# Unsigned-Long/slam-tricks

Hardware: AMD Instinct MI355X
Metric: LM iterations/sec + residuals/sec, 1k-cam/100k-pt BA (higher is better)
Workload: dtype f64

## Files before the change

slam-tricks_amd/csrc/dense_chol.hip:

```cpp
#include <algorithm>
#include <atomic>
#include <cstdlib>
#include <map>
#include <mutex>
#include <queue>
#include <string>
#include <vector>

#include "common.hpp"

namespace stba {

constexpr int NB = CHOL_NB;
#ifndef MEGA_WAIT_SLEEP
#define MEGA_WAIT_SLEEP 1
#endif
#ifndef MEGA_POLL_SLEEP
#define MEGA_POLL_SLEEP 16
#endif

typedef double double4v __attribute__((ext_vector_type(4)));

__global__ void chol_pad_kernel(double* __restrict__ A, int lda, int n, const double* __restrict__ rhs) {
    const int r = n + blockIdx.x;
// ... 455 lines not shown
        for (int p = 0; p < 2; ++p)
#pragma unroll
            for (int h = 0; h < 2; ++h) {
                const int row = lrow + 16 * (w + 4 * p);
                const int k = 2 * (lkp + 4 * h);
                if (p < PA) ga[p < PA ? p : 0][h] = *reinterpret_cast<const double2*>(&A[(size_t)(row_i + row) * lda + k0 + kc * 16 + k]);
                gb[p][h] = *reinterpret_cast<const double2*>(&A[(size_t)(row_j + row) * lda + k0 + kc * 16 + k]);
            }
    };
    auto lstore = [&](int buf) {
#pragma unroll
        for (int p = 0; p < 2; ++p)
#pragma unroll
            for (int h = 0; h < 2; ++h) {
                const int rb = w + 4 * p;
                const int k = 2 * (lkp + 4 * h);
                if (p < PA) {
                    const int posa = (((k >> 2) * RBA + rb) << 6) + ((k & 3) << 4) + lrow;
                    sA[buf][posa] = ga[p < PA ? p : 0][h].x;
                    sA[buf][posa + 16] = ga[p < PA ? p : 0][h].y;
                }
                const int posb = (((k >> 2) * 8 + rb) << 6) + ((k & 3) << 4) + lrow;
                sB[buf][posb] = gb[p][h].x;
                sB[buf][posb + 16] = gb[p][h].y;
            }
    };
    gload(0);
    lstore(0);
    __syncthreads();
    constexpr int KC = NB / 16;
    for (int kc = 0; kc < KC; ++kc) {
        const int buf = kc & 1;
        if (kc + 1 < KC) gload(kc + 1);
#pragma unroll
        for (int kq = 0; kq < 4; ++kq) {
            double a[MB], b[NBK];
#pragma unroll
            for (int m = 0; m < MB; ++m) a[m] = -sA[buf][((kq * RBA + wr * MB + m) << 6) + lane];
#pragma unroll
            for (int n = 0; n < NBK; ++n) b[n] = sB[buf][((kq * 8 + wc * NBK + n) << 6) + lane];
#pragma unroll
            for (int m = 0; m < MB; ++m)
#pragma unroll
                for (int n = 0; n < NBK; ++n)
                    acc[m][n] = __builtin_amdgcn_mfma_f64_16x16x4f64(a[m], b[n], acc[m][n], 0, 0, 0);
        }
        if (kc + 1 < KC) lstore(buf ^ 1);
        __syncthreads();
    }
#pragma unroll
    for (int m = 0; m < MB; ++m)
#pragma unroll
        for (int n = 0; n < NBK; ++n)
#pragma unroll
            for (int r = 0; r < 4; ++r) {
                const int row = row_i + wr * (MB * 16) + m * 16 + (lane >> 4) + 4 * r;
                const int col = row_j + wc * (NBK * 16) + n * 16 + (lane & 15);
                A[(size_t)row * lda + col] = acc[m][n][r];
            }
}

static void launch_syrk(double* A, int lda, int k0, int tile_mode, int tiles128, hipStream_t st) {
    const bool use64 = tiles128 < 1000000;
    if (use64) hipLaunchKernelGGL(chol_syrk_kernel<64>, dim3(2 * tiles128), dim3(256), 0, st, A, lda, k0, tile_mode);
    else hipLaunchKernelGGL(chol_syrk_kernel<128>, dim3(tiles128), dim3(256), 0, st, A, lda, k0, tile_mode);
}

enum { TASK_D = 0, TASK_T = 1, TASK_TI = 2, TASK_U = 3, TASK_UQ = 4, TASK_TU = 5 };

constexpr int MEGA_MAX_Q = 16;
struct MegaArgs {
    double* A; int lda; int n; int nblk;
    const int4* tasks;
    int nq;
    int lstart[MEGA_MAX_Q + 1];
    signed char xcc_queue[16];
    int* sync;
    double* linv; size_t linv_stride;
    double* vbuf; int nwide;
    long long spin_limit;
    int* flag;
    long long* trace;
};
constexpr int MEGA_SYNC_HDR = MEGA_MAX_Q + 1;
constexpr int MEGA_ABORT = MEGA_MAX_Q;
constexpr int MEGA_SMEM_BYTES = 128 * 1024;
constexpr int MEGA_PREDRAW_NB = 2;

__device__ __forceinline__ int xcc_id() {
    unsigned v;
    asm volatile("s_getreg_b32 %0, hwreg(HW_REG_XCC_ID)" : "=s"(v));
    return (int)(v & 15u);
}
__global__ void xcc_probe_kernel(int* out) {
    if (threadIdx.x == 0) out[blockIdx.x] = xcc_id();
}

template <int TM, int KCH = 16>
__device__ __forceinline__ void syrk_tile512(double* __restrict__ A, int lda, int k0, int row_i, int row_j,
                                             double* smem, int t, int kchunks = NB / 16) {
    constexpr int WR = (TM == 128) ? 2 : 1, WC = 8 / WR;
    constexpr int MB = TM / (16 * WR);
    constexpr int NBK = 8 / WC;
    constexpr int RBA = TM / 16;
    constexpr int SA = TM * KCH, SB = 128 * KCH, NH = KCH / 8;
    double* sA = smem;
    double* sB = smem + 2 * SA;
    const int lane = t & 63, w = t >> 6;
    const int wr = w / WC, wc = w % WC;
    double4v acc[MB][NBK];
#pragma unroll
    for (int m = 0; m < MB; ++m)
#pragma unroll
        for (int n = 0; n < NBK; ++n)
#pragma unroll
            for (int r = 0; r < 4; ++r) {
                const int row = row_i + wr * (MB * 16) + m * 16 + (lane >> 4) + 4 * r;
                const int col = row_j + wc * (NBK * 16) + n * 16 + (lane & 15);
                acc[m][n][r] = A[(size_t)row * lda + col];
            }
    double2 ga[NH], gb[NH];
    const int lrow = lane & 15, lkp = lane >> 4;
    const bool stage_a = (RBA == 8) ? true : (w < RBA);
    auto gload = [&](int kc) {
#pragma unroll
        for (int h = 0; h < NH; ++h) {
            const int row = lrow + 16 * w;
            const int k = 2 * (lkp + 4 * h);
            if (stage_a) ga[h] = *reinterpret_cast<const double2*>(&A[(size_t)(row_i + row) * lda + k0 + kc * KCH + k]);
            gb[h] = *reinterpret_cast<const double2*>(&A[(size_t)(row_j + row) * lda + k0 + kc * KCH + k]);
        }
    };
    auto lstore = [&](int buf) {
#pragma unroll
        for (int h = 0; h < NH; ++h) {
            const int k = 2 * (lkp + 4 * h);
            if (stage_a) {
                const int posa = (((k >> 2) * RBA + w) << 6) + ((k & 3) << 4) + lrow;
                sA[buf * SA + posa] = -ga[h].x;
                sA[buf * SA + posa + 16] = -ga[h].y;
            }
            const int posb = (((k >> 2) * 8 + w) << 6) + ((k & 3) << 4) + lrow;
            sB[buf * SB + posb] = gb[h].x;
            sB[buf * SB + posb + 16] = gb[h].y;
        }
    };
    gload(0);
    lstore(0);
    __syncthreads();
    const int KC = kchunks * 16 / KCH;
    auto chunk = [&](int kc, int buf) {
        if (kc + 1 < KC) gload(kc + 1);
#pragma unroll
        for (int kq = 0; kq < KCH / 4; ++kq) {
            double a[MB], b[NBK];
#pragma unroll
            for (int m = 0; m < MB; ++m) a[m] = sA[buf * SA + (((kq * RBA + wr * MB + m) << 6) + lane)];
#pragma unroll
            for (int n = 0; n < NBK; ++n) b[n] = sB[buf * SB + (((kq * 8 + wc * NBK + n) << 6) + lane)];
#pragma unroll
            for (int m = 0; m < MB; ++m)
#pragma unroll
                for (int n = 0; n < NBK; ++n)
                    acc[m][n] = __builtin_amdgcn_mfma_f64_16x16x4f64(a[m], b[n], acc[m][n], 0, 0, 0);
        }
        if (kc + 1 < KC) lstore(buf ^ 1);
// ... 364 lines not shown
    v.nblk = a.nblk;
    v.nrow = a.nblk + 4 * a.nwide;
    v.abortf = a.sync + MEGA_ABORT;
    v.dflag = a.sync + MEGA_SYNC_HDR;
    v.tuflag = v.dflag + a.nblk;
    v.tudone = v.tuflag + a.nblk;
    v.tflag = v.tudone + a.nblk;
    v.ver = v.tflag + a.nblk * v.nrow;
    return v;
}
__device__ __forceinline__ int mega_ldf(const int* p) { return __hip_atomic_load(p, __ATOMIC_RELAXED, __HIP_MEMORY_SCOPE_AGENT); }
__device__ __forceinline__ bool mega_ready(const MegaView& v, const int4 d, bool& tu_dset) {
    const int type = d.x & 0xff, b = d.y, ti = d.z, tj = d.w;
    const int nblk = v.nblk, nrow = v.nrow;
    auto first_panel = [&](int i) { return i < nblk ? 0 : i - nblk; };
    if (type == TASK_D) return mega_ldf(&v.ver[b * nblk + b]) >= 4 * b;
    if (type == TASK_T) {
        const int ve = mega_ldf(&v.ver[ti * nblk + b]), df = mega_ldf(&v.dflag[b]);
        return (ve >= 4 * (b - first_panel(ti))) & (df >= 1);
    }
    if (type == TASK_TI) return mega_ldf(&v.dflag[b]) >= 1;
    if (type == TASK_TU) {
        const int v0 = mega_ldf(&v.ver[(b + 1) * nblk + b]), v1 = mega_ldf(&v.ver[(b + 1) * nblk + b + 1]), df = mega_ldf(&v.dflag[b]);
        tu_dset = df >= 1;
        return (v0 >= 4 * b) & (v1 >= 4 * b);
    }
    const int i = (type == TASK_UQ) ? (ti >> 2) : ti;
    const int nbp = max(1, (d.x >> 16) & 0xff);
    const int f0 = mega_ldf(&v.tflag[b * nrow + i]), f1 = mega_ldf(&v.tflag[b * nrow + tj]), ve = mega_ldf(&v.ver[i * nblk + tj]);
    return (f0 >= 4) & (f1 >= 4) & (ve >= 4 * (b - nbp + 1 - first_panel(i)));
}

struct MegaTicket {
    int mine = -1;
    int4 md;
    bool done = false;
    int m_raw = 0;
    bool m_pending = false;
};
__device__ __forceinline__ int mega_next_task(const MegaArgs& a, const MegaView& v, MegaTicket& tk, int* ticket, int lbeg, int lend, int lane,
                                              bool& ok, bool& tu_dset, long long& t_poll) {
    t_poll = a.trace ? wall_clock64() : 0;
    ok = true;
    if (tk.mine < 0 && !tk.done) {
        if (!tk.m_pending && lane == 0) tk.m_raw = lbeg + atomicAdd(ticket, 1);
        tk.m_pending = false;
        tk.mine = __builtin_amdgcn_readfirstlane(tk.m_raw);
        if (tk.mine >= lend) { tk.mine = -1; tk.done = true; }
        else tk.md = a.tasks[tk.mine];
    }
    int pick = -2;
    if (tk.mine >= 0) {
        const long long t0 = wall_clock64();
        for (;;) {
            if (mega_ready(v, tk.md, tu_dset)) { pick = tk.mine; tk.mine = -1; break; }
            if (mega_ldf(v.abortf) != 0) { ok = false; pick = -1; break; }
            if (wall_clock64() - t0 > a.spin_limit) {
                __hip_atomic_store(v.abortf, 1, __ATOMIC_RELAXED, __HIP_MEMORY_SCOPE_AGENT);
                ok = false; pick = -1;
                break;
            }
            __builtin_amdgcn_s_sleep(MEGA_POLL_SLEEP);
        }
    }
    asm volatile("buffer_inv sc1\n\ts_waitcnt vmcnt(0)" ::: "memory");
    return pick;
}

__global__ __launch_bounds__(512) void chol_mega_kernel(MegaArgs a) {
    extern __shared__ __attribute__((aligned(16))) double smem[];
    __shared__ int s_task, s_ok, s_dset;
    const int t = threadIdx.x;
    const int nblk = a.nblk;
    const MegaView v = mega_view(a);
    int* abortf = v.abortf;
    int* dflag = v.dflag;
    int* tuflag = v.tuflag;
    const int nrow = v.nrow;
    int* tflag = v.tflag;
    int* ver = v.ver;
    auto tile_ptr = [&](int i, int j, int& ld) -> double* {
        if (i < nblk) { ld = a.lda; return a.A + (size_t)i * NB * a.lda + (size_t)j * NB; }
        const int p = i - nblk, qw = p >> 2;
        ld = 4 * NB;
        return a.vbuf + (size_t)qw * (4 * NB) * (4 * NB) + (size_t)(p & 3) * NB * (4 * NB) + (size_t)(j - 4 * qw) * NB;
    };
    auto first_panel = [&](int i) { return i < nblk ? 0 : i - nblk; };
    const int q = a.xcc_queue[xcc_id()];
    if (q < 0) return;
    int* ticket = a.sync + q;
    const int lbeg = a.lstart[q], lend = a.lstart[q + 1];
    MegaTicket tk;
    for (;;) {
        if (t < 64) {
            bool ok, tu_dset = false;
            long long t_poll;
            const int pick = mega_next_task(a, v, tk, ticket, lbeg, lend, t, ok, tu_dset, t_poll);
            if (t == 0) {
                if (a.trace && pick >= 0) {
                    a.trace[8 * (size_t)pick] = blockIdx.x; a.trace[8 * (size_t)pick + 1] = t_poll;
                    a.trace[8 * (size_t)pick + 2] = wall_clock64();
                }
                s_dset = tu_dset ? 1 : 0;
                s_task = pick;
                s_ok = ok ? 1 : 0;
            }
            if (!tk.done && pick >= 0 && (tk.md.x & 0xff) != TASK_TU && ((tk.md.x >> 16) & 0xff) <= MEGA_PREDRAW_NB) {
                if (t == 0) tk.m_raw = lbeg + atomicAdd(ticket, 1);
                tk.m_pending = true;
            }
        }
        __syncthreads();
        if (!s_ok) {
            if (t == 0) atomicExch(a.flag, CHOL_FLAG_TIMEOUT);
            break;
        }
        const int task = s_task;
        if (task < 0) break;
        const int4 d = a.tasks[task];
        const int type = d.x & 0xff, b = d.y, ti = d.z, tj = d.w;
        const int k0 = b * NB;
        int tt = t;
        asm volatile("" : "+v"(tt));
        double* li = a.linv + (size_t)b * a.linv_stride;
        long long* ph = a.trace ? a.trace + 8 * (size_t)task + 4 : nullptr;
        if (type == TASK_D) {
            diag_block2<true>(a.A, a.lda, k0, a.n, a.flag, li + NB * NB, smem, tt, ph);
        } else if (type == TASK_T) {
            const int lane = tt & 63, w = tt >> 6;
            int ldr;
            const bool active = (tj == 0) || (w < 4);
            const int row_in_tile = (tj == 0 ? 16 * w : 64 * (tj - 1) + 16 * (w & 3)) + (lane & 15);
            double* rowp = tile_ptr(ti, b, ldr) + (size_t)row_in_tile * ldr;
            if (!trsm_task512(rowp, false, 0, NB, a.A + (size_t)k0 * a.lda + k0, a.lda, li + NB * NB, smem, tt, ph, &dflag[b], abortf, &s_ok,
                              a.spin_limit, true, active)) {
                if (t == 0) atomicExch(a.flag, CHOL_FLAG_TIMEOUT);
                break;
            }
        } else if (type == TASK_TI) {
            const int lane = tt & 63, w = tt >> 6;
            const int nv = min(NB, (a.lda - 1) - k0);
            int ldr = NB;
            double* base = li;
            if (b < 4 * a.nwide) base = tile_ptr(nblk + b, b, ldr);
            double* rowp = base + (size_t)(16 * w + (lane & 15)) * ldr;
            if (!trsm_task512(rowp, true, 16 * w, nv, a.A + (size_t)k0 * a.lda + k0, a.lda, li + NB * NB, smem, tt, ph, &dflag[b], abortf, &s_ok,
                              a.spin_limit, true)) {
                if (t == 0) atomicExch(a.flag, CHOL_FLAG_TIMEOUT);
                break;
            }
        } else if (type == TASK_U) {
            if (ti < nblk) {
                const int nbp = max(1, (d.x >> 16) & 0xff);
                syrk_tile512<128>(a.A, a.lda, k0 - (nbp - 1) * NB, ti * NB, tj * NB, smem, tt, nbp * (NB / 16));
            } else {
                int ldc, ldi, ldj;
                double* Cb = tile_ptr(ti, tj, ldc);
                const double* Pi = tile_ptr(ti, b, ldi);
                const double* Pj = tile_ptr(tj, b, ldj);
                syrk_tile512_gen<128>(Cb, ldc, Pi, ldi, Pj, ldj, b == first_panel(ti), smem, tt);
            }
        } else if (type == TASK_TU) {
            const bool tu_ok = (tj == 2)
                ? tu4_task512(a.A, a.lda, k0, b + 1, ti, li + NB * NB, smem, tt, ph, &tuflag[b], &ver[(b + 1) * nblk + b + 1], &dflag[b], abortf, &s_ok,
                              a.spin_limit, s_dset != 0)
                : tu_task512(a.A, a.lda, k0, b + 1, ti, li + NB * NB, smem, tt, ph, &tuflag[b], &v.tudone[b], &ver[(b + 1) * nblk + b + 1], &dflag[b], abortf, &s_ok,
                             a.spin_limit, s_dset != 0);
            if (!tu_ok) {
// ... 109 lines not shown
            }
        for (int i = b + 2; i < NBK; ++i) {
            if (b >= THALF_FROM) {
                idT[(size_t)b * NBK + i] = add(TASK_T, b, i, 1, 10.0 * b + 6 + 1e-3 * i);
                idT2[(size_t)b * NBK + i] = add(TASK_T, b, i, 2, 10.0 * b + 6 + 1e-3 * i + 5e-4);
                nodes[(size_t)idT[(size_t)b * NBK + i]].dur = nodes[(size_t)idT2[(size_t)b * NBK + i]].dur = THALF_DUR * DUR[TASK_T];
            } else idT[(size_t)b * NBK + i] = add(TASK_T, b, i, 0, 10.0 * b + 6 + 1e-3 * i);
            if (i <= b + 1 + QROWS || b >= QFROM) {
                for (int q = 0; q < 4; ++q)
                    idUq[((size_t)b * NBK + i) * 4 + q] = add(TASK_UQ, b, i * 4 + q, b + 1, 10.0 * (b + 1) + 2 + 1e-3 * i);
            } else {
                idUq[((size_t)b * NBK + i) * 4] = add(TASK_U, b, i, b + 1, 10.0 * (b + 1) + 2 + 1e-3 * i);
            }
        }
        for (int j = b + 2; j < NBK; ++j) {
            const int lim = j - 2 - BLAG;
            int BJ = BATCH;
            if (FAR > 0 && BATCH > 1 && j - ((b / (2 * BATCH)) * 2 * BATCH + 2 * BATCH - 1) > FAR) BJ = 2 * BATCH;
            const int b0 = (BJ <= 1 || b > lim) ? b : (b / BJ) * BJ, last = (BJ <= 1 || b > lim) ? b : std::min(b0 + BJ - 1, lim);
            if (b != last) continue;
            const int nb = b - b0 + 1;
            for (int i = j; i < NBK; ++i) {
                if (i == j && j == b + 2 && b >= DQ_FROM) {
                    for (int q = 0; q < 4; ++q) {
                        const int id = add(TASK_UQ, b, i * 4 + q, j, 10.0 * j + 1 + 1e-3 * q);
                        idUd[(size_t)b * 4 + q] = id;
                        if (q == 0) idU[((size_t)b * NBK + i) * NBK + j] = id;
                    }
                    continue;
                }
                const int id = add(TASK_U, b, i, j, 10.0 * j + 3 + 1e-3 * i + 1e-6 * b);
                nodes[(size_t)id].tk.x |= nb << 16;
                nodes[(size_t)id].dur += (nb - 1) * DUR_K;
                for (int bb = b0; bb <= b; ++bb) idU[((size_t)bb * NBK + i) * NBK + j] = id;
            }
        }
    }
    auto dep = [&](int from, int to) {
        if (from < 0 || to < 0) return;
        nodes[(size_t)from].succ.push_back(to);
        nodes[(size_t)to].indeg++;
    };
    for (int b = 0; b < NBK; ++b) {
        const int d = idD[(size_t)b];
        if (b > 0)
            for (int q = 0; q < ntu(b - 1); ++q) dep(idTU[(size_t)(b - 1) * MEGA_NTU + q], d);
        dep(d, idTI[(size_t)b]);
        if (b + 1 < NBK)
            for (int q = 0; q < ntu(b); ++q) {
                const int tu = idTU[(size_t)b * MEGA_NTU + q];
                dep(d, tu);
                if (b > 0) {
                    for (int q2 = 0; q2 < 4; ++q2) dep(idUq[((size_t)(b - 1) * NBK + (b + 1)) * 4 + q2], tu);
                    dep(idU[((size_t)(b - 1) * NBK + (b + 1)) * NBK + (b + 1)], tu);
                    for (int q2 = 1; q2 < 4; ++q2) dep(idUd[(size_t)(b - 1) * 4 + q2], tu);
                }
            }
        for (int i = b + 2; i < NBK; ++i) {
            const int t = idT[(size_t)b * NBK + i], t2 = idT2[(size_t)b * NBK + i];
            dep(d, t); dep(d, t2);
            if (b > 0)
                for (int q2 = 0; q2 < 4; ++q2) { const int uu = idUq[((size_t)(b - 1) * NBK + i) * 4 + q2]; dep(uu, t); dep(uu, t2); }
            for (int q = 0; q < 4; ++q) {
                const int uq = idUq[((size_t)b * NBK + i) * 4 + q];
                if (uq < 0) continue;
                dep(t, uq); dep(t2, uq);
                for (int q2 = 0; q2 < ntu(b); ++q2) dep(idTU[(size_t)b * MEGA_NTU + q2], uq);
                if (b > 0) dep(idU[((size_t)(b - 1) * NBK + i) * NBK + (b + 1)], uq);
            }
        }
        for (int j = b + 2; j < NBK; ++j)
            for (int i = j; i < NBK; ++i) {
                const int u0 = idU[((size_t)b * NBK + i) * NBK + j];
                if (nodes[(size_t)u0].tk.y != b) continue;
                const bool split = (nodes[(size_t)u0].tk.x & 0xff) == TASK_UQ;
                for (int q2 = 0; q2 < (split ? 4 : 1); ++q2) {
                    const int u = split ? idUd[(size_t)b * 4 + q2] : u0;
                    for (auto* v : {&idT, &idT2}) { dep((*v)[(size_t)b * NBK + i], u); if (j != i) dep((*v)[(size_t)b * NBK + j], u); }
                    const int nbp = split ? 1 : std::max(1, (nodes[(size_t)u].tk.x >> 16) & 0xff);
                    if (b - nbp >= 0) dep(idU[((size_t)(b - nbp) * NBK + i) * NBK + j], u);
                }
            }
    }
    for (int qw = 0; qw < nwide; ++qw)
        for (int v = 0; v < 4; ++v) {
            const int pnl = 4 * qw + v, iv = NBK + pnl;
            std::vector<int> xdone(4, -1);
            xdone[(size_t)v] = idTI[(size_t)pnl];
            for (int j = v + 1; j < 4; ++j) {
                const int bj = 4 * qw + j;
                int prev = -1;
                for (int k = pnl; k < bj; ++k) {
                    const int u = add(TASK_U, k, iv, bj, 10.0 * NBK + bj);
                    dep(xdone[(size_t)(k - 4 * qw)], u);
                    if (bj == k + 1) { for (int q2 = 0; q2 < ntu(k); ++q2) dep(idTU[(size_t)k * MEGA_NTU + q2], u); }
                    else for (auto* v : {&idT, &idT2}) dep((*v)[(size_t)k * NBK + bj], u);
                    dep(prev, u);
                    prev = u;
                }
                const int tv = add(TASK_T, bj, iv, 0, 10.0 * NBK + bj);
                dep(idD[(size_t)bj], tv);
                dep(prev, tv);
                xdone[(size_t)j] = tv;
            }
        }
    static const double BLW = knob_double("STBA_MEGA_BLEVEL", 1.0);
    if (BLW > 0.0) {
        std::vector<int> indeg2(nodes.size()), topo;
        topo.reserve(nodes.size());
        for (size_t k = 0; k < nodes.size(); ++k) { indeg2[k] = nodes[k].indeg; if (indeg2[k] == 0) topo.push_back((int)k); }
        for (size_t h = 0; h < topo.size(); ++h)
            for (int sidx : nodes[(size_t)topo[h]].succ)
                if (--indeg2[(size_t)sidx] == 0) topo.push_back(sidx);
        std::vector<double> bl(nodes.size(), 0.0);
        for (size_t h = topo.size(); h-- > 0;) {
            const int k = topo[h];
            double m = 0.0;
            for (int sidx : nodes[(size_t)k].succ) m = std::max(m, bl[(size_t)sidx]);
            bl[(size_t)k] = nodes[(size_t)k].dur + m;
        }
        for (size_t k = 0; k < nodes.size(); ++k) nodes[k].prio = nodes[k].prio * (1.0 - BLW) * 5.0 - BLW * bl[k];
    }
    static const double ADV_D = knob_double("STBA_MEGA_ADV_D", 0.0), ADV_TU = knob_double("STBA_MEGA_ADV_TU", 0.0);
    typedef std::pair<double, int> PI;
    typedef std::priority_queue<PI, std::vector<PI>, std::greater<PI>> Heap;
    std::vector<Heap> ready_h((size_t)nl);
    Heap events;
    std::vector<std::vector<double>> idle_since((size_t)nl, std::vector<double>((size_t)mach.wg, 0.0));
    double now = 0.0;
    struct Pick { double key, start; int node; };
    std::vector<std::vector<Pick>> order((size_t)nl);
    auto push_ready = [&](int k) { ready_h[(size_t)nodes[(size_t)k].q].push(PI(nodes[(size_t)k].prio, k)); };
    for (int k = 0; k < (int)nodes.size(); ++k)
        if (nodes[(size_t)k].indeg == 0) push_ready(k);
    double makespan = 0.0;
    std::vector<double> tiles_in((size_t)std::max(1, n_gpus), 0.0);
    for (;;) {
        for (int l = 0; l < nl; ++l) {
            std::vector<double>& idl = idle_since[(size_t)l];
            Heap& hb = ready_h[(size_t)l];
            while (!idl.empty() && !hb.empty()) {
                const int k = hb.top().second;
                hb.pop();
                Node& nd = nodes[(size_t)k];
                const int ty = nd.tk.x & 0xff;
                const double adv = ty == TASK_D ? ADV_D : ty == TASK_TU ? ADV_TU : 0.0;
                order[(size_t)l].push_back({idl.back() - adv, now, k});
                idl.pop_back();
                nd.start = now;
                events.push(PI(now + nd.dur, k));
            }
        }
        if (events.empty()) break;
        const PI ev = events.top();
        events.pop();
        now = ev.first;
        if (ev.second < 0) {
            const int k = -(ev.second + 1);
            nodes[(size_t)k].ready = now;
            push_ready(k);
            continue;
        }
        makespan = now;
        const Node& nd = nodes[(size_t)ev.second];
        idle_since[(size_t)nd.q].push_back(now);
        const int g0 = gpu_of(nd.q);
        unsigned sent_to = 0;
        for (int sidx : nd.succ) {
            Node& sn = nodes[(size_t)sidx];
            double at = now;
            const int g1 = gpu_of(sn.q);
            if (g1 != g0) {
                at += shard->hop_us + shard->tile_us;
                shard->cross_edges += 1.0;
                if (!(sent_to >> g1 & 1u)) { sent_to |= 1u << g1; tiles_in[(size_t)g1] += 1.0; }
            }
            if (at > sn.avail) { sn.avail = at; sn.last_pred = ev.second; }
            if (--sn.indeg == 0) {
                if (sn.avail <= now) { sn.ready = now; push_ready(sidx); }
                else events.push(PI(sn.avail, -(sidx + 1)));
            }
        }
    }
    if (makespan_out) *makespan_out = makespan;
    if (shard) shard->tiles_in_max = *std::max_element(tiles_in.begin(), tiles_in.end());
    if (knob_str("STBA_MEGA_SIMDBG")) {
        static const char* NM[6] = {"D", "T", "TI", "U", "Uq", "TU"};
// ... 36 lines not shown
    mega_build_tasks(nblk, m, tasks, lstart.data(), nullptr, &ms);
    return ms;
}

void chol_shard_model(int nblk, int n_gpus, int n_xcd, int wg_per_q, int rows_per_group, double hop_us, double tile_us, double* out3) {
    std::vector<int4> tasks;
    std::vector<int> lstart((size_t)n_gpus * n_xcd + 1);
    MegaShardModel sh;
    sh.n_gpus = n_gpus; sh.rows_per_group = rows_per_group; sh.hop_us = hop_us; sh.tile_us = tile_us;
    double ms = 0.0;
    MegaMachine m;
    m.nq = n_gpus * n_xcd; m.wg = wg_per_q;
    mega_build_tasks(nblk, m, tasks, lstart.data(), nullptr, &ms, 0, &sh);
    out3[0] = ms; out3[1] = sh.cross_edges; out3[2] = sh.tiles_in_max;
}

int chol_shard_row_owner(int row, int n_gpus, int rows_per_group) { return (row / std::max(1, rows_per_group)) % std::max(1, n_gpus); }

constexpr int BWD_ROW_CHUNKS = 8;
__global__ __launch_bounds__(1024) void chol_bwd_step_kernel(double* __restrict__ A, int lda, int k0, int has_next,
                                                             const double* __restrict__ Xinv, double* __restrict__ x) {
    __shared__ double xs[NB];
    __shared__ double part[BWD_ROW_CHUNKS][NB];
    __shared__ double ybuf[NB];
    const int t = threadIdx.x;
    const int kn = k0 + NB;
    const int nvn = has_next ? min(NB, (lda - 1) - kn) : 0;
    constexpr int RPC = NB / BWD_ROW_CHUNKS;
    const int rchunk = t >> 7, c = t & 127;
    const int c0 = (blockIdx.x > 0) ? (blockIdx.x - 1) * NB : k0;
    double lv[RPC];
#pragma unroll
    for (int j = 0; j < RPC; ++j) lv[j] = 0.0;
    if (has_next) {
        const double* col = A + (size_t)(kn + rchunk * RPC) * lda + c0 + c;
#pragma unroll
        for (int j = 0; j < RPC; ++j) lv[j] = col[(size_t)j * lda];
    }
    const int i = t >> 3, p8 = t & 7;
    double xv[16];
    double y_own = 0.0;
    const int nv = min(NB, (lda - 1) - k0);
    if (blockIdx.x == 0) {
        const double* xr = Xinv + (size_t)i * NB + p8 * 16;
#pragma unroll
        for (int j = 0; j < 16; ++j) xv[j] = xr[j];
        if (t < NB) y_own = (t < nv) ? A[(size_t)(lda - 1) * lda + k0 + t] : 0.0;
    }
    double y_upd = 0.0;
    if (blockIdx.x > 0 && t < NB) y_upd = A[(size_t)(lda - 1) * lda + c0 + t];
    if (t < NB) xs[t] = (t < nvn) ? x[kn + t] : 0.0;
    __syncthreads();
    double s = 0.0;
#pragma unroll
    for (int j = 0; j < RPC; ++j) s = fma(lv[j], xs[rchunk * RPC + j], s);
    part[rchunk][c] = s;
    __syncthreads();
    if (blockIdx.x > 0) {
        if (t < NB) {
            double acc = 0.0;
#pragma unroll
            for (int q = 0; q < BWD_ROW_CHUNKS; ++q) acc += part[q][t];
            A[(size_t)(lda - 1) * lda + c0 + t] = y_upd - acc;
        }
        return;
    }
    if (t < NB) {
        double yv = y_own;
#pragma unroll
        for (int q = 0; q < BWD_ROW_CHUNKS; ++q) yv -= part[q][t];
        ybuf[t] = (t < nv) ? yv : 0.0;
    }
    __syncthreads();
    double r = 0.0;
#pragma unroll
    for (int j = 0; j < 16; ++j) r = fma(xv[j], ybuf[p8 * 16 + j], r);
    r += __shfl_xor(r, 1, 64);
    r += __shfl_xor(r, 2, 64);
    r += __shfl_xor(r, 4, 64);
    if (p8 == 0) x[k0 + i] = (i < nv) ? r : 0.0;
}

template <int RPC>
__global__ __launch_bounds__(1024) void chol_bwd_apply_kernel(double* __restrict__ A, int lda, int src_row0, const double* __restrict__ x) {
    __shared__ double xs[32 * RPC];
    __shared__ double part[32][33];
    const int t = threadIdx.x, rc = t >> 5, c = t & 31;
    const int c0 = blockIdx.x * 32;
    const double* col = A + (size_t)(src_row0 + rc * RPC) * lda + c0 + c;
    double lv[RPC];
#pragma unroll
    for (int j = 0; j < RPC; ++j) lv[j] = col[(size_t)j * lda];
    for (int e = t; e < 32 * RPC; e += 1024) xs[e] = x[src_row0 + e];
    double yv = 0.0;
    if (t < 32) yv = A[(size_t)(lda - 1) * lda + c0 + t];
    __syncthreads();
    double s = 0.0;
#pragma unroll
    for (int j = 0; j < RPC; ++j) s = fma(lv[j], xs[rc * RPC + j], s);
    part[rc][c] = s;
    __syncthreads();
    if (t < 32) {
        double acc = 0.0;
#pragma unroll
        for (int q = 0; q < 32; ++q) acc += part[q][t];
        A[(size_t)(lda - 1) * lda + c0 + t] = yv - acc;
    }
}
constexpr int BWD_SOLVE_ROWS = 8;
__global__ __launch_bounds__(32 * BWD_SOLVE_ROWS) void chol_bwd_wide_solve_kernel(const double* __restrict__ A, int lda, const double* __restrict__ V, int row0,
                                                                                  double* __restrict__ x) {
    __shared__ double ys[4 * NB];
    const int t = threadIdx.x, r = blockIdx.x * BWD_SOLVE_ROWS + (t >> 5), cc = t & 31;
    const bool live = (cc >> 3) >= (r >> 7);
    double v[16];
    if (live) {
        const double* vr = V + (size_t)r * (4 * NB) + 16 * cc;
#pragma unroll
        for (int j = 0; j < 16; ++j) v[j] = vr[j];
    }
    for (int e = t; e < 4 * NB; e += 32 * BWD_SOLVE_ROWS) ys[e] = A[(size_t)(lda - 1) * lda + row0 + e];
    __syncthreads();
    double s = 0.0;
    if (live) {
#pragma unroll
        for (int j = 0; j < 16; ++j) s = fma(v[j], ys[16 * cc + j], s);
    }
    s += __shfl_xor(s, 1, 64);
    s += __shfl_xor(s, 2, 64);
    s += __shfl_xor(s, 4, 64);
    s += __shfl_xor(s, 8, 64);
    s += __shfl_xor(s, 16, 64);
    if (cc == 0) x[row0 + r] = s;
}

struct MegaDevice {
    std::mutex m;
    bool probed = false;
    int ncu = 0, nq = 0;
    signed char xcc_queue[16];
    hipEvent_t last = nullptr;
    hipStream_t last_stream = nullptr;
    int cooldown = 0;
};
static MegaDevice& mega_device(int dev) {
    static std::mutex mm;
    static std::map<int, MegaDevice> devs;
    std::lock_guard<std::mutex> g(mm);
    return devs[dev];
}

static int mega_device_init(MegaDevice& D, hipStream_t st) {
    if (D.probed) return STBA_OK;
    int dev = 0;
    hipDeviceProp_t prop;
    STBA_HIP(hipGetDevice(&dev));
    STBA_HIP(hipGetDeviceProperties(&prop, dev));
    D.ncu = prop.multiProcessorCount;
    int* probe = nullptr;
    std::vector<int> h((size_t)D.ncu);
    STBA_HIP(hipMalloc(reinterpret_cast<void**>(&probe), h.size() * sizeof(int)));
    hipLaunchKernelGGL(xcc_probe_kernel, dim3(D.ncu), dim3(512), 0, st, probe);
    hipError_t e = hipMemcpyAsync(h.data(), probe, h.size() * sizeof(int), hipMemcpyDeviceToHost, st);
    if (e == hipSuccess) e = hipStreamSynchronize(st);
    (void)hipFree(probe);
    STBA_HIP(e);
    for (int i = 0; i < 16; ++i) D.xcc_queue[i] = -1;
    int per_xcc[16] = {0};
    D.nq = 0;
    for (int x : h) {
        if (D.xcc_queue[x & 15] < 0) D.xcc_queue[x & 15] = (signed char)D.nq++;
        per_xcc[x & 15]++;
    }
    for (int i = 0; i < 16; ++i)
        if (D.xcc_queue[i] >= 0 && per_xcc[i] < MEGA_NTU)
            return fail(STBA_ERR_HIP, "chol: fewer than 10 workgroups per XCD (the TU tasks of a step need one each)");
    if (!D.last) STBA_HIP(hipEventCreateWithFlags(&D.last, hipEventDisableTiming));
    D.probed = true;
    return STBA_OK;
}

void chol_forget_stream(hipStream_t st) {
    for (int dev = 0; dev < 64; ++dev) {
        MegaDevice& D = mega_device(dev);
        std::lock_guard<std::mutex> g(D.m);
        if (D.last_stream == st) D.last_stream = nullptr;
        if (dev > 0 && !D.probed) break;
    }
}

static std::atomic<int> g_timeouts{0};
static std::atomic<long long> g_spin_override{0};
void chol_set_spin_limit_us(double us) { g_spin_override.store(us > 0.0 ? std::max(1LL, (long long)(us * 100.0)) : 0LL); }
void chol_note_timeout() {
    g_timeouts.fetch_add(1);
    int dev = 0;
    if (hipGetDevice(&dev) != hipSuccess) return;
    MegaDevice& D = mega_device(dev);
    std::lock_guard<std::mutex> g(D.m);
    D.cooldown = 64;
}
void chol_count_timeout() { g_timeouts.fetch_add(1); }
void chol_note_peer_timeout() {
    int dev = 0;
    if (hipGetDevice(&dev) != hipSuccess) return;
    MegaDevice& D = mega_device(dev);
    std::lock_guard<std::mutex> g(D.m);
    D.cooldown = 64;
}
int chol_timeout_count() { return g_timeouts.load(); }

enum { CHOL_PERSISTENT = 0, CHOL_STAGES = 1 };

static int chol_run(double* A, int lda, int n, double* x_dev, int* flag_dev, hipStream_t st, CholProfile* prof,
                    hipEvent_t mid_event = nullptr, int schedule = CHOL_PERSISTENT, hipEvent_t pre_event = nullptr) {
    if (lda % NB != 0 || lda < n + 1) return fail(STBA_ERR_INVALID_ARGUMENT, "chol: bad padded dimension");
    const int nblk = lda / NB;
    int cur_dev = 0;
    STBA_HIP(hipGetDevice(&cur_dev));
    if (!prof && schedule == CHOL_PERSISTENT) {
        MegaDevice& D = mega_device(cur_dev);
        std::lock_guard<std::mutex> g(D.m);
        if (D.cooldown > 0) { --D.cooldown; schedule = CHOL_STAGES; }
    }
    const bool stages = prof != nullptr || schedule == CHOL_STAGES;
    constexpr size_t LINV_STRIDE = (size_t)NB * NB + 8 * 256;
    struct MegaPlan {
        int nblk = 0, nwide = -1, ntasks = 0;
        int lstart[MEGA_MAX_Q + 1] = {0};
        int4* tasks = nullptr; int* sync = nullptr; size_t sync_ints = 0;
        double makespan_us = 0.0;
        std::vector<float> sim_start;
    };
    struct DevWs { double* linv = nullptr; int linv_blocks = 0; double* vbuf = nullptr; int vbuf_blocks = 0; MegaPlan plan; };
    static thread_local std::map<int, DevWs> ws_by_dev;
    DevWs& ws = ws_by_dev[cur_dev];
    double*& linv = ws.linv;
    int& linv_blocks = ws.linv_blocks;
    if (linv_blocks < nblk) {
        if (linv) (void)hipFree(linv);
        linv = nullptr; linv_blocks = 0;
        STBA_HIP(hipMalloc(reinterpret_cast<void**>(&linv), (size_t)nblk * LINV_STRIDE * sizeof(double)));
        linv_blocks = nblk;
    }
    const int nwide = stages ? 0 : (nblk - 1) / 4;
    if (ws.vbuf_blocks < nwide) {
        if (ws.vbuf) (void)hipFree(ws.vbuf);
        ws.vbuf = nullptr; ws.vbuf_blocks = 0;
        STBA_HIP(hipMalloc(reinterpret_cast<void**>(&ws.vbuf), (size_t)nwide * 16 * NB * NB * sizeof(double)));
        ws.vbuf_blocks = nwide;
    }
    static DeviceOnce diag_attr;
    STBA_TRY(diag_attr.run([]() -> int {
        STBA_HIP(hipFuncSetAttribute(reinterpret_cast<const void*>(chol_diag_kernel), hipFuncAttributeMaxDynamicSharedMemorySize, (int)sizeof(Diag2Smem)));
        return STBA_OK;
    }));
    auto launch_panel_diag = [&](int b, hipStream_t s_) {
        double* li = linv + (size_t)b * LINV_STRIDE;
        hipLaunchKernelGGL(chol_diag_kernel, dim3(1), dim3(512), sizeof(Diag2Smem), s_, A, lda, b * NB, n, flag_dev, li + NB * NB);
    };
    auto launch_panel_trsm = [&](int b, hipStream_t s_) {
        double* li = linv + (size_t)b * LINV_STRIDE;
        const int groups = (nblk - b - 1) * (NB / 16);
        hipLaunchKernelGGL(chol_trsm_kernel, dim3(groups + NB / 16), dim3(64), 0, s_, A, lda, b * NB, groups, li, li + NB * NB);
    };
    std::vector<hipEvent_t> ev;
    if (prof) {
        ev.resize((size_t)nblk * 4 + 2);
        for (auto& e : ev) STBA_HIP(hipEventCreate(&e));
        memset(prof, 0, sizeof *prof);
    }
    auto mark = [&](size_t k) -> int { if (prof) STBA_HIP(hipEventRecord(ev[k], st)); return STBA_OK; };
    if (stages) {
        {
            MegaDevice& D = mega_device(cur_dev);
            std::lock_guard<std::mutex> dev_lock(D.m);
            if (!D.last) STBA_HIP(hipEventCreateWithFlags(&D.last, hipEventDisableTiming));
            if (D.last_stream != nullptr && D.last_stream != st) {
                STBA_HIP(hipEventRecord(D.last, D.last_stream));
                STBA_HIP(hipStreamWaitEvent(st, D.last, 0));
            }
            D.last_stream = st;
        }
        STBA_HIP(hipMemsetAsync(flag_dev, 0, sizeof(int), st));
        for (int b = 0; b < nblk; ++b) {
            const int k0 = b * NB;
            const int mt = nblk - b - 1;
            STBA_TRY(mark(4 * (size_t)b + 0));
            launch_panel_diag(b, st);
            STBA_TRY(mark(4 * (size_t)b + 1));
            launch_panel_trsm(b, st);
            STBA_TRY(mark(4 * (size_t)b + 2));
            if (mt > 0) launch_syrk(A, lda, k0, 0, mt * (mt + 1) / 2, st);
            STBA_TRY(mark(4 * (size_t)b + 3));
            if (mt > 0 && prof) {
                const double m = std::max(0, n - (k0 + NB));
                prof->syrk_flops += m * (m + 1.0) * NB;
                prof->syrk_flops_padded += (double)(mt * (mt + 1) / 2) * 2.0 * NB * NB * NB;
                prof->syrk_launches += 1;
            }
        }
    } else {
        MegaDevice& D = mega_device(cur_dev);
        std::lock_guard<std::mutex> dev_lock(D.m);
        STBA_TRY(mega_device_init(D, st));
        MegaPlan& plan = ws.plan;
        if (plan.nblk != nblk || plan.nwide != nwide) {
            if (plan.tasks) (void)hipFree(plan.tasks);
            if (plan.sync) (void)hipFree(plan.sync);
            plan = MegaPlan();
            MegaMachine mach;
            mach.nq = D.nq;
            mach.wg = std::max(MEGA_NTU, D.ncu / D.nq);
            std::vector<int4> tasks;
            mega_build_tasks(nblk, mach, tasks, plan.lstart, &plan.sim_start, &plan.makespan_us, nwide);
            STBA_HIP(hipMalloc(reinterpret_cast<void**>(&plan.tasks), tasks.size() * sizeof(int4)));
            STBA_HIP(hipMemcpy(plan.tasks, tasks.data(), tasks.size() * sizeof(int4), hipMemcpyHostToDevice));
            plan.sync_ints = MEGA_SYNC_HDR + 3 * (size_t)nblk + 2 * (size_t)nblk * (nblk + 4 * nwide);
            STBA_HIP(hipMalloc(reinterpret_cast<void**>(&plan.sync), plan.sync_ints * sizeof(int)));
            plan.ntasks = (int)tasks.size();
            plan.nblk = nblk; plan.nwide = nwide;
        }
        hipLaunchKernelGGL(chol_reset_kernel, dim3((unsigned)((plan.sync_ints + 255) / 256)), dim3(256), 0, st, plan.sync, (int)plan.sync_ints, flag_dev);
        MegaArgs ma;
        ma.A = A; ma.lda = lda; ma.n = n; ma.nblk = nblk;
        ma.tasks = plan.tasks; ma.nq = D.nq; ma.sync = plan.sync;
        memcpy(ma.lstart, plan.lstart, sizeof ma.lstart);
        memcpy(ma.xcc_queue, D.xcc_queue, sizeof ma.xcc_queue);
        ma.linv = linv; ma.linv_stride = LINV_STRIDE; ma.flag = flag_dev;
        ma.vbuf = ws.vbuf; ma.nwide = nwide;
        ma.spin_limit = (long long)std::max(25e3, 40.0 * plan.makespan_us) * 100LL;
        if (g_spin_override.load() > 0) ma.spin_limit = g_spin_override.load();
        static const char* TRACE = knob_str("STBA_MEGA_TRACE");
        ma.trace = nullptr;
        if (TRACE) STBA_HIP(hipMalloc(reinterpret_cast<void**>(&ma.trace), (size_t)plan.ntasks * 8 * sizeof(long long)));
        struct TraceGuard { long long*& p; ~TraceGuard() { if (p) { (void)hipFree(p); p = nullptr; } } } trace_guard{ma.trace};
        static DeviceOnce attr_set;
        STBA_TRY(attr_set.run([]() -> int {
            STBA_HIP(hipFuncSetAttribute(reinterpret_cast<const void*>(chol_mega_kernel),
                                         hipFuncAttributeMaxDynamicSharedMemorySize, MEGA_SMEM_BYTES));
            return STBA_OK;
        }));
        if (D.last_stream != nullptr && D.last_stream != st) {
            STBA_HIP(hipEventRecord(D.last, D.last_stream));
            STBA_HIP(hipStreamWaitEvent(st, D.last, 0));
        }
        if (pre_event) STBA_HIP(hipEventRecord(pre_event, st));
        hipLaunchKernelGGL(chol_mega_kernel, dim3(D.ncu), dim3(512), MEGA_SMEM_BYTES, st, ma);
        D.last_stream = st;
        if (TRACE) {
            std::vector<long long> h((size_t)plan.ntasks * 8);
            std::vector<int4> ht((size_t)plan.ntasks);
            STBA_HIP(hipStreamSynchronize(st));
            STBA_HIP(hipMemcpy(h.data(), ma.trace, h.size() * sizeof(long long), hipMemcpyDeviceToHost));
            STBA_HIP(hipMemcpy(ht.data(), plan.tasks, ht.size() * sizeof(int4), hipMemcpyDeviceToHost));
            if (FILE* f = fopen(TRACE, "wb")) {
                fwrite(&plan.ntasks, sizeof(int), 1, f);
                fwrite(ht.data(), sizeof(int4), ht.size(), f);
                fwrite(h.data(), sizeof(long long), h.size(), f);
                fwrite(plan.sim_start.data(), sizeof(float), plan.sim_start.size(), f);
                fclose(f);
            }
        }
    }
    STBA_TRY(mark((size_t)nblk * 4));
    if (mid_event) STBA_HIP(hipEventRecord(mid_event, st));
    for (int b = nblk - 1; b >= 4 * nwide; --b) {
        const int k0 = b * NB;
        const int has_next = (b < nblk - 1) ? 1 : 0;
        const int grid = 1 + (has_next ? b : 0);
        hipLaunchKernelGGL(chol_bwd_step_kernel, dim3(grid), dim3(1024), 0, st, A, lda, k0, has_next, linv + (size_t)b * LINV_STRIDE, x_dev);
    }
    for (int qw = nwide - 1; qw >= 0; --qw) {
        const int row0 = qw * 4 * NB;
        if (qw == nwide - 1) hipLaunchKernelGGL(chol_bwd_apply_kernel<4>, dim3((row0 + 4 * NB) / 32), dim3(1024), 0, st, A, lda, row0 + 4 * NB, x_dev);
        else hipLaunchKernelGGL(chol_bwd_apply_kernel<16>, dim3((row0 + 4 * NB) / 32), dim3(1024), 0, st, A, lda, row0 + 4 * NB, x_dev);
        hipLaunchKernelGGL(chol_bwd_wide_solve_kernel, dim3(4 * NB / BWD_SOLVE_ROWS), dim3(32 * BWD_SOLVE_ROWS), 0, st, A, lda, ws.vbuf + (size_t)qw * 16 * NB * NB, row0, x_dev);
    }
    STBA_TRY(mark((size_t)nblk * 4 + 1));
    STBA_HIP(hipGetLastError());
    if (prof) {
        STBA_HIP(hipStreamSynchronize(st));
        float ms = 0.f;
        for (int b = 0; b < nblk; ++b) {
            (void)hipEventElapsedTime(&ms, ev[4 * (size_t)b + 0], ev[4 * (size_t)b + 1]); prof->ms_diag += ms;
            (void)hipEventElapsedTime(&ms, ev[4 * (size_t)b + 1], ev[4 * (size_t)b + 2]); prof->ms_trsm += ms;
            (void)hipEventElapsedTime(&ms, ev[4 * (size_t)b + 2], ev[4 * (size_t)b + 3]); prof->ms_syrk += ms;
        }
        (void)hipEventElapsedTime(&ms, ev[(size_t)nblk * 4], ev[(size_t)nblk * 4 + 1]); prof->ms_bwd = ms;
        for (auto& e : ev) (void)hipEventDestroy(e);
    }
    return STBA_OK;
}

size_t chol_spd_inverse_workspace_doubles(int np) { return (size_t)(np / NB) * ((size_t)NB * NB + 8 * 256); }
int chol_spd_inverse_dev(double* W, int ldw, int np, int n_real, int* flag_dev, double* work, hipStream_t st) {
    if (np % NB != 0 || ldw != 2 * np || np <= 0) return fail(STBA_ERR_INVALID_ARGUMENT, "chol_spd_inverse_dev: bad dimensions");
    constexpr size_t LINV_STRIDE = (size_t)NB * NB + 8 * 256;
    static DeviceOnce diag_attr;
    STBA_TRY(diag_attr.run([]() -> int {
        STBA_HIP(hipFuncSetAttribute(reinterpret_cast<const void*>(chol_diag_kernel), hipFuncAttributeMaxDynamicSharedMemorySize, (int)sizeof(Diag2Smem)));
        return STBA_OK;
    }));
    STBA_HIP(hipMemsetAsync(flag_dev, 0, sizeof(int), st));
    const int nblk = ldw / NB;
    for (int b = 0; b < np / NB; ++b) {
        double* li = work + (size_t)b * LINV_STRIDE;
        const int mt = nblk - b - 1;
        hipLaunchKernelGGL(chol_diag_kernel, dim3(1), dim3(512), sizeof(Diag2Smem), st, W, ldw, b * NB, n_real, flag_dev, li + NB * NB);
        const int groups = mt * (NB / 16);
        hipLaunchKernelGGL(chol_trsm_kernel, dim3(groups + NB / 16), dim3(64), 0, st, W, ldw, b * NB, groups, li, li + NB * NB);
        launch_syrk(W, ldw, b * NB, 0, mt * (mt + 1) / 2, st);
    }
    STBA_HIP(hipGetLastError());
    return STBA_OK;
}

__global__ __launch_bounds__(512) void yyt_tile_kernel(const double* __restrict__ Y, size_t ldy, double* __restrict__ S, int lda, int ntiles, int nsplit,
                                                       int chunks_per_split, int chunks_total, double* __restrict__ ws, const int2* __restrict__ tile_ij,
                                                       int per_xcd) {
    extern __shared__ __attribute__((aligned(16))) double smem[];
    const int w = (int)(blockIdx.x % 8) * per_xcd + (int)(blockIdx.x / 8);
    if (blockIdx.x / 8 >= (unsigned)per_xcd || w >= ntiles * nsplit) return;
    const int split = w / ntiles, tile = w % ntiles;
    const int I = tile_ij[tile].x, J = tile_ij[tile].y;
    const int c0 = split * chunks_per_split, c1 = min(chunks_total, c0 + chunks_per_split);
    double* Cb = (nsplit == 1) ? S + (size_t)I * NB * lda + (size_t)J * NB : ws + ((size_t)split * ntiles + tile) * NB * NB;
    const int ldc = (nsplit == 1) ? lda : NB;
    if (c1 <= c0) {
        for (int e = threadIdx.x; e < NB * NB; e += 512) Cb[(size_t)(e / NB) * ldc + e % NB] = 0.0;
        return;
    }
    syrk_tile512_gen<128>(Cb, ldc, Y + (size_t)I * NB * ldy + (size_t)c0 * 16, ldy, Y + (size_t)J * NB * ldy + (size_t)c0 * 16, ldy, true, smem,
                          threadIdx.x, c1 - c0);
}
__global__ __launch_bounds__(256) void yyt_reduce_kernel(const double* __restrict__ ws, int ntiles, int nsplit, double* __restrict__ S, int lda,
                                                         const int2* __restrict__ tile_ij) {
    const int tile = blockIdx.x / (NB * NB / 256);
    const int e = (blockIdx.x % (NB * NB / 256)) * 256 + threadIdx.x;
    const int I = tile_ij[tile].x, J = tile_ij[tile].y;
    const int r = e / NB, c = e % NB;
    double s = 0.0;
    if (nsplit == 1) s = S[((size_t)I * NB + r) * lda + (size_t)J * NB + c];
    else for (int k = 0; k < nsplit; ++k) s += ws[((size_t)k * ntiles + tile) * NB * NB + e];
    if (I == J && c > r) s = 0.0;
    S[((size_t)I * NB + r) * lda + (size_t)J * NB + c] = s;
}
static int yyt_splits(int ntiles, int chunks_total) {
    int ns = (4096 + ntiles - 1) / ntiles;
    ns = std::min(ns, 64);
    ns = std::min(ns, std::max(1, chunks_total / 8));
    return std::max(1, ns);
}
size_t chol_yyt_workspace_doubles(int lda, size_t kcols) {
    const int nb = lda / NB, ntiles = nb * (nb + 1) / 2;
    const int ns = yyt_splits(ntiles, (int)(kcols / 16));
    return ns == 1 ? 0 : (size_t)ns * ntiles * NB * NB;
}
static int yyt_tile_list(int nb, int2** out_dev) {
    static std::mutex m;
// ... 62 lines not shown
```

Before: 370.6.

## Widen inverse panel buffer to cover next wide group and fuse backward apply/solve

Doubles the leading dimension of the per-group inverse buffer so each wide group's V block also spans the next four panels. The mega-kernel task graph gains extra update tasks that fold those cross-group terms in during factorization, gated behind a diagonal task near the end so they fill idle time. The backward solve can then merge the apply and wide-solve steps for non-last groups into one kernel, which removes launches and a pass over the triangular factor. In exchange the factorization does more work and needs twice the vbuf memory.

```diff
diff --git a/slam-tricks_amd/csrc/dense_chol.hip b/slam-tricks_amd/csrc/dense_chol.hip
--- a/slam-tricks_amd/csrc/dense_chol.hip
+++ b/slam-tricks_amd/csrc/dense_chol.hip
@@ -561,6 +561,8 @@
     int* flag;
     long long* trace;
 };
+constexpr int VB_LD = 8 * NB;
+constexpr size_t VB_BLOCK = (size_t)(4 * NB) * VB_LD;
 constexpr int MEGA_SYNC_HDR = MEGA_MAX_Q + 1;
 constexpr int MEGA_ABORT = MEGA_MAX_Q;
 constexpr int MEGA_SMEM_BYTES = 128 * 1024;
@@ -1091,8 +1093,8 @@
     auto tile_ptr = [&](int i, int j, int& ld) -> double* {
         if (i < nblk) { ld = a.lda; return a.A + (size_t)i * NB * a.lda + (size_t)j * NB; }
         const int p = i - nblk, qw = p >> 2;
-        ld = 4 * NB;
-        return a.vbuf + (size_t)qw * (4 * NB) * (4 * NB) + (size_t)(p & 3) * NB * (4 * NB) + (size_t)(j - 4 * qw) * NB;
+        ld = VB_LD;
+        return a.vbuf + (size_t)qw * VB_BLOCK + (size_t)(p & 3) * NB * VB_LD + (size_t)(j - 4 * qw) * NB;
     };
     auto first_panel = [&](int i) { return i < nblk ? 0 : i - nblk; };
     const int q = a.xcc_queue[xcc_id()];
@@ -1368,6 +1370,7 @@
                 }
             }
     }
+    static const int W_HOLD = std::max(0, knob_int("STBA_MEGA_W_HOLD", 10));
     for (int qw = 0; qw < nwide; ++qw)
         for (int v = 0; v < 4; ++v) {
             const int pnl = 4 * qw + v, iv = NBK + pnl;
@@ -1389,6 +1392,19 @@
                 dep(prev, tv);
                 xdone[(size_t)j] = tv;
             }
+            if (qw + 1 < nwide)
+                for (int bj = 4 * qw + 4; bj < 4 * qw + 8; ++bj) {
+                    int prev = -1;
+                    for (int k = pnl; k < 4 * qw + 4; ++k) {
+                        const int u = add(TASK_U, k, iv, bj, 10.0 * NBK + bj);
+                        dep(xdone[(size_t)(k - 4 * qw)], u);
+                        if (bj == k + 1) { for (int q2 = 0; q2 < ntu(k); ++q2) dep(idTU[(size_t)k * MEGA_NTU + q2], u); }
+                        else for (auto* v : {&idT, &idT2}) dep((*v)[(size_t)k * NBK + bj], u);
+                        if (prev < 0 && W_HOLD > 0) dep(idD[(size_t)std::min(NBK - 1, std::max(4 * qw + 4, NBK - W_HOLD))], u);
+                        dep(prev, u);
+                        prev = u;
+                    }
+                }
         }
     static const double BLW = knob_double("STBA_MEGA_BLEVEL", 1.0);
     if (BLW > 0.0) {
@@ -1591,11 +1607,9 @@
 }
 
 template <int RPC>
-__global__ __launch_bounds__(1024) void chol_bwd_apply_kernel(double* __restrict__ A, int lda, int src_row0, const double* __restrict__ x) {
-    __shared__ double xs[32 * RPC];
-    __shared__ double part[32][33];
-    const int t = threadIdx.x, rc = t >> 5, c = t & 31;
-    const int c0 = blockIdx.x * 32;
+__device__ __forceinline__ void bwd_apply32(double* __restrict__ A, int lda, int src_row0, const double* __restrict__ x, int c0, int t,
+                                            double* __restrict__ xs, double (*part)[33]) {
+    const int rc = t >> 5, c = t & 31;
     const double* col = A + (size_t)(src_row0 + rc * RPC) * lda + c0 + c;
     double lv[RPC];
 #pragma unroll
@@ -1615,6 +1629,11 @@
         for (int q = 0; q < 32; ++q) acc += part[q][t];
         A[(size_t)(lda - 1) * lda + c0 + t] = yv - acc;
     }
+}
+__global__ __launch_bounds__(1024) void chol_bwd_apply_kernel(double* __restrict__ A, int lda, int src_row0, const double* __restrict__ x) {
+    __shared__ double xs[NB];
+    __shared__ double part[32][33];
+    bwd_apply32<NB / 32>(A, lda, src_row0, x, blockIdx.x * 32, threadIdx.x, xs, part);
 }
 constexpr int BWD_SOLVE_ROWS = 8;
 __global__ __launch_bounds__(32 * BWD_SOLVE_ROWS) void chol_bwd_wide_solve_kernel(const double* __restrict__ A, int lda, const double* __restrict__ V, int row0,
@@ -1624,7 +1643,7 @@
     const bool live = (cc >> 3) >= (r >> 7);
     double v[16];
     if (live) {
-        const double* vr = V + (size_t)r * (4 * NB) + 16 * cc;
+        const double* vr = V + (size_t)r * VB_LD + 16 * cc;
 #pragma unroll
         for (int j = 0; j < 16; ++j) v[j] = vr[j];
     }
@@ -1641,6 +1660,41 @@
     s += __shfl_xor(s, 8, 64);
     s += __shfl_xor(s, 16, 64);
     if (cc == 0) x[row0 + r] = s;
+}
+__global__ __launch_bounds__(1024) void chol_bwd_wide_step_kernel(double* __restrict__ A, int lda, const double* __restrict__ VW, int row0,
+                                                                  double* __restrict__ x) {
+    constexpr int NSOLVE = 4 * NB / BWD_SOLVE_ROWS;
+    __shared__ double vec[8 * NB];
+    __shared__ double part[32][33];
+    const int t = threadIdx.x;
+    if ((int)blockIdx.x >= NSOLVE) {
+        bwd_apply32<4 * NB / 32>(A, lda, row0 + 4 * NB, x, ((int)blockIdx.x - NSOLVE) * 32, t, vec, part);
+        return;
+    }
+    const int rl = t >> 7, r = blockIdx.x * BWD_SOLVE_ROWS + rl, cc = t & 127;
+    const bool live = (cc >> 4) >= (r >> 7);
+    const double* vr = VW + (size_t)r * VB_LD + 8 * cc;
+    double4v v0 = {0.0, 0.0, 0.0, 0.0}, v1 = {0.0, 0.0, 0.0, 0.0};
+    if (live) { v0 = gld4(vr); v1 = gld4(vr + 4); }
+    if (t < 4 * NB) vec[t] = A[(size_t)(lda - 1) * lda + row0 + t];
+    else vec[t] = x[row0 + t];
+    __syncthreads();
+    double s = 0.0;
+    if (live) {
+#pragma unroll
+        for (int j = 0; j < 4; ++j) s = fma(v0[j], vec[8 * cc + j], s);
+#pragma unroll
+        for (int j = 0; j < 4; ++j) s = fma(v1[j], vec[8 * cc + 4 + j], s);
+    }
+    s += __shfl_xor(s, 1, 64);
+    s += __shfl_xor(s, 2, 64);
+    s += __shfl_xor(s, 4, 64);
+    s += __shfl_xor(s, 8, 64);
+    s += __shfl_xor(s, 16, 64);
+    s += __shfl_xor(s, 32, 64);
+    if ((t & 63) == 0) part[rl][(t >> 6) & 1] = s;
+    __syncthreads();
+    if (t < BWD_SOLVE_ROWS) x[row0 + blockIdx.x * BWD_SOLVE_ROWS + t] = part[t][0] + part[t][1];
 }
 
 struct MegaDevice {
@@ -1756,7 +1810,7 @@
     if (ws.vbuf_blocks < nwide) {
         if (ws.vbuf) (void)hipFree(ws.vbuf);
         ws.vbuf = nullptr; ws.vbuf_blocks = 0;
-        STBA_HIP(hipMalloc(reinterpret_cast<void**>(&ws.vbuf), (size_t)nwide * 16 * NB * NB * sizeof(double)));
+        STBA_HIP(hipMalloc(reinterpret_cast<void**>(&ws.vbuf), (size_t)nwide * VB_BLOCK * sizeof(double)));
         ws.vbuf_blocks = nwide;
     }
     static DeviceOnce diag_attr;
@@ -1882,9 +1936,13 @@
     }
     for (int qw = nwide - 1; qw >= 0; --qw) {
         const int row0 = qw * 4 * NB;
-        if (qw == nwide - 1) hipLaunchKernelGGL(chol_bwd_apply_kernel<4>, dim3((row0 + 4 * NB) / 32), dim3(1024), 0, st, A, lda, row0 + 4 * NB, x_dev);
-        else hipLaunchKernelGGL(chol_bwd_apply_kernel<16>, dim3((row0 + 4 * NB) / 32), dim3(1024), 0, st, A, lda, row0 + 4 * NB, x_dev);
-        hipLaunchKernelGGL(chol_bwd_wide_solve_kernel, dim3(4 * NB / BWD_SOLVE_ROWS), dim3(32 * BWD_SOLVE_ROWS), 0, st, A, lda, ws.vbuf + (size_t)qw * 16 * NB * NB, row0, x_dev);
+        const double* vw = ws.vbuf + (size_t)qw * VB_BLOCK;
+        if (qw == nwide - 1) {
+            hipLaunchKernelGGL(chol_bwd_apply_kernel, dim3((row0 + 4 * NB) / 32), dim3(1024), 0, st, A, lda, row0 + 4 * NB, x_dev);
+            hipLaunchKernelGGL(chol_bwd_wide_solve_kernel, dim3(4 * NB / BWD_SOLVE_ROWS), dim3(32 * BWD_SOLVE_ROWS), 0, st, A, lda, vw, row0, x_dev);
+        } else {
+            hipLaunchKernelGGL(chol_bwd_wide_step_kernel, dim3(4 * NB / BWD_SOLVE_ROWS + row0 / 32), dim3(1024), 0, st, A, lda, vw, row0, x_dev);
+        }
     }
     STBA_TRY(mark((size_t)nblk * 4 + 1));
     STBA_HIP(hipGetLastError());
```

New measurement: 370.2. No clear change (-0.1%).
